# nsbuitrago/vfind

Measured on NVIDIA B200. Metric: reads/sec, higher is better.
Workload: dtype int32

## Files before the change

include/vfind_b200.h:

```cpp
#ifndef VFIND_B200_H
#define VFIND_B200_H

#include <stddef.h>
#include <stdint.h>

#ifdef __cplusplus
extern "C" {
#endif

#define VFB_ABI_VERSION 1

typedef enum vfb_status {
    VFB_OK = 0,
    VFB_ERR_VALUE = 1,
    VFB_ERR_IO = 2,
    VFB_ERR_FORMAT = 3,
    VFB_ERR_CUDA = 4,
    VFB_ERR_ARG = 5,
    VFB_ERR_NOMEM = 6
} vfb_status;

#define VFB_NONE 0xFFFFFFFFu

typedef struct vfb_params {
// ... 196 lines not shown
typedef struct vfb_dp_layout_info {
    int32_t packed;
    int32_t max_edits;
    int32_t accept_bound;
    uint32_t lcap;
    int32_t S0, LB, XB;
    int32_t c_eopen, c_eext, c_fopen, c_fext;
    int32_t hmask, lowmask, lenmask;
    int32_t neg_e, neg_f;
    int32_t w_match, w_mismatch, w_wild;
} vfb_dp_layout_info;

int vfb_debug_dp_layout(int32_t match_score, int32_t mismatch_score, int32_t gap_open_penalty, int32_t gap_extend_penalty,
                        uint32_t adapter_len, double accept_alignment, int32_t dp_mode, vfb_dp_layout_info *out);

int vfb_host_alloc(void **p, uint64_t bytes);
int vfb_host_free(void *p);

int vfb_pinned_pool_trim(void);
int vfb_device_pool_trim(void);

#ifdef __cplusplus
}
#endif
#endif
```

vfind_b200/csrc/api.cu:

```cuda
#include <cmath>
#include <cstdio>
#include <cstdlib>
#include <cstring>
#include <sched.h>
#include <string>
#include <thread>
#include <vector>

#include "hash.h"
#include "synth.h"
#include "ctx.cuh"

namespace vfb {

thread_local std::string g_error;
thread_local uint64_t g_launches = 0;

void set_error(const std::string &msg) { g_error = msg; }

int cuda_fail(cudaError_t e, const char *what, const char *file, int line)
{
    char buf[512];
    snprintf(buf, sizeof buf, "CUDA error %d (%s) at %s:%d: %s", (int)e, cudaGetErrorString(e), file, line, what);
    g_error = buf;
// ... 610 lines not shown
    if (c->st_parse) cudaStreamSynchronize(c->st_parse);
    for (auto &ln : c->lanes) { if (ln.st) cudaStreamSynchronize(ln.st); if (ln.st_dp) cudaStreamSynchronize(ln.st_dp); }
    for (auto &s : c->slots) {
        s.d_text.release(); s.d_spans.release(); s.h_text.release(); s.h_spans.release();
        if (s.copied) cudaEventDestroy(s.copied);
        for (auto &ev : s.computed) if (ev) cudaEventDestroy(ev);
    }
    for (auto &g : c->seg) {
        g.text.release(); g.z.release(); g.members.release(); g.spans.release();
        if (g.parsed) cudaEventDestroy(g.parsed);
        if (g.inflated) cudaEventDestroy(g.inflated);
        if (g.copied) cudaEventDestroy(g.copied);
        for (auto &ev : g.computed) if (ev) cudaEventDestroy(ev);
    }
    for (auto &ln : c->lanes) {
        DevBuf *lb[] = {&ln.d_start, &ln.d_end, &ln.d_list_a, &ln.d_list_b, &ln.d_fb_a, &ln.d_fb_b, &ln.d_c32, &ln.d_t64, &ln.d_keys,
                        &ln.d_koff, &ln.d_klen, &ln.d_khash, &ln.d_owner, &ln.d_wins, &ln.d_bestkey, &ln.d_cbval, &ln.d_fb2};
        for (auto *b : lb) b->release();
        if (ln.done) cudaEventDestroy(ln.done);
        if (ln.ev_scanned) cudaEventDestroy(ln.ev_scanned);
        if (ln.ev_aligned) cudaEventDestroy(ln.ev_aligned);
        if (ln.st) cudaStreamDestroy(ln.st);
        if (ln.st_dp) cudaStreamDestroy(ln.st_dp);
    }
    if (c->ev_fork) cudaEventDestroy(c->ev_fork);
    if (c->ev_k4) cudaEventDestroy(c->ev_k4);
    DevBuf *bufs[] = {&c->d_code_pre, &c->d_code_suf, &c->d_generic_scratch, &c->d_diag_exact_pre, &c->d_diag_exact_suf, &c->d_diag_score_pre,
                      &c->d_diag_len_pre, &c->d_diag_score_suf, &c->d_diag_len_suf, &c->t_slots,
                      &c->t_row_hash, &c->t_row_off, &c->t_row_len, &c->t_row_slot, &c->t_arena, &c->t_counters, &c->t_row_count,
                      &c->m_part_rows, &c->m_part_keys, &c->m_cursors, &c->m_chunk_off, &c->m_send, &c->m_recv,
                      &c->d_aligned_text, &c->d_span_sum,
                      &c->x_block_bytes, &c->x_block_rows, &c->x_offsets, &c->x_counts, &c->x_data,
// ... 144 lines not shown
    const uint64_t span_bytes_upper = span_len_ub;
    if (!text_bytes_hint) text_bytes_hint = span_bytes_upper;
    int rc;
    if (n == 0) return VFB_OK;
    const int li = c->n_lanes > 1 ? (int)(c->lane_seq++ & 1u) : 0;
    Lane &ln = c->lanes[li];
    cudaStream_t st = c->n_lanes > 1 ? ln.st : c->st_compute;
    if (lanes_used) *lanes_used |= 1u << li;
    const bool prof = c->profiling;
    if ((rc = ln.d_start.ensure((size_t)n * 4))) return rc;
    if ((rc = ln.d_end.ensure((size_t)n * 4))) return rc;
    if (c->align_pre) { if ((rc = ln.d_list_a.ensure((size_t)n * 4))) return rc; if ((rc = ln.d_fb_a.ensure((size_t)n * 4))) return rc; }
    if (c->align_suf) { if ((rc = ln.d_list_b.ensure((size_t)n * 4))) return rc; if ((rc = ln.d_fb_b.ensure((size_t)n * 4))) return rc; }
    const uint64_t key_bytes_ub = (c->prm.skip_translation ? span_bytes_upper : span_bytes_upper / 3) + 16ull * n;
    if ((rc = ln.d_keys.ensure(key_bytes_ub))) return rc;
    if ((rc = ln.d_koff.ensure((size_t)n * 8))) return rc;
    if ((rc = ln.d_klen.ensure((size_t)n * 4))) return rc;
    if ((rc = ln.d_khash.ensure((size_t)n * 8))) return rc;
    if ((rc = ln.d_owner.ensure((size_t)n * 4))) return rc;
    if (c->win_k_pre >= 0 || c->win_k_suf >= 0) {
        const uint32_t cap = n < 0x3FFFFFFFu ? n * 2u + 1024u : 0x7FFFFFFFu;
        if ((rc = ln.d_wins.ensure((size_t)cap * dpw_item_bytes()))) return rc;
        ln.win_cap = (uint32_t)(ln.d_wins.cap / dpw_item_bytes());
        if (c->prm.debug_win_cap > 0 && (uint32_t)c->prm.debug_win_cap < ln.win_cap) ln.win_cap = (uint32_t)c->prm.debug_win_cap;
        if ((rc = ln.d_bestkey.ensure((size_t)n * 8))) return rc;
        if ((rc = ln.d_cbval.ensure((size_t)n * 8))) return rc;
        if ((rc = ln.d_fb2.ensure((size_t)n * 4))) return rc;
    }
    const bool diag = c->prm.diagnostics != 0;
    if (diag) {
// ... 46 lines not shown
    ++g_launches;
    if (split) {
        VFB_CUDA(cudaEventRecord(ln.ev_aligned, sd));
        VFB_CUDA(cudaStreamWaitEvent(st, ln.ev_aligned, 0));
    }

    KeyJob kj;
    kj.text = d_text; kj.spans = d_spans;
    kj.start = ln.d_start.as<uint32_t>(); kj.end = ln.d_end.as<uint32_t>();
    kj.n_reads = n; kj.text_bytes = text_bytes_hint; kj.skip_translation = c->prm.skip_translation;
    kj.keys = ln.d_keys.as<uint8_t>(); kj.koff = ln.d_koff.as<uint64_t>();
    kj.key_cursor = ln.d_t64.as<unsigned long long>() + T_KEYBYTES;
    kj.klen = ln.d_klen.as<uint32_t>(); kj.khash = ln.d_khash.as<uint64_t>();
    kj.hash_bits = c->prm.debug_hash_bits;
    kj.flank_bytes = (uint32_t)(c->prefix.size() + c->suffix.size());
    bool k4_waited = false;
    InsertJob ij;
    ij.keys = kj.keys; ij.klen = kj.klen; ij.khash = kj.khash; ij.kcount = nullptr; ij.koff = kj.koff;
    ij.key_stride = 0; ij.n_keys = n; ij.owner_slot = ln.d_owner.as<uint32_t>();
    int frc = -1;
    if (c->fused_count && c->ub_rows > 0) {
        if (c->n_lanes > 1 && c->k4_pending) { VFB_CUDA(cudaStreamWaitEvent(st, c->ev_k4, 0)); k4_waited = true; }
        frc = launch_keys_count(kj, c->tab, ln.d_c32.as<uint32_t>() + C_NMISS, st);
        if (frc > 0) return frc;
        if (frc == VFB_OK) { ij.n_keys_dev = ln.d_c32.as<uint32_t>() + C_NMISS; ++c->stats.fused_batches; }
    }
    if (frc != VFB_OK && (rc = launch_keys(kj, st))) return rc;
    if (prof) VFB_CUDA(cudaEventRecord(pev[6], st));

    if (c->n_lanes > 1 && c->k4_pending && !k4_waited) VFB_CUDA(cudaStreamWaitEvent(st, c->ev_k4, 0));
    if ((rc = launch_insert(c->tab, ij, st))) return rc;
    if ((rc = snaps_push(c, n, key_bytes_ub, st))) return rc;
    if (c->n_lanes > 1) {
        VFB_CUDA(cudaEventRecord(c->ev_k4, st));
// ... 929 lines not shown
    DpLayout l;
    uint32_t lcap = 0;
    int K = -1;
    out->packed = plan_packed_dp(sc, adapter_len, out->accept_bound, dp_mode != 1, &l, &lcap, &K) ? 1 : 0;
    out->max_edits = out->packed ? K : -1;
    if (!out->packed) return VFB_OK;
    out->S0 = l.S0; out->LB = l.LB; out->XB = l.XB;
    out->c_eopen = l.c_eopen; out->c_eext = l.c_eext; out->c_fopen = l.c_fopen; out->c_fext = l.c_fext;
    out->hmask = l.hmask; out->lowmask = l.lowmask; out->lenmask = l.lenmask;
    out->neg_e = l.neg_e; out->neg_f = l.neg_f;
    out->w_match = l.w_match; out->w_mismatch = l.w_mismatch; out->w_wild = l.w_wild;
    out->lcap = lcap;
    return VFB_OK;
}

int vfb_host_alloc(void **p, uint64_t bytes)
{
    if (!p) { set_error("null argument"); return VFB_ERR_ARG; }
    VFB_CUDA(cudaMallocHost(p, bytes ? bytes : 1));
    return VFB_OK;
}

int vfb_host_free(void *p)
{
    if (p) VFB_CUDA(cudaFreeHost(p));
    return VFB_OK;
}

int vfb_pinned_pool_trim(void)
{
// ... 12 lines not shown
```

vfind_b200/csrc/ctx.cuh:

```cuda
#pragma once
#include <chrono>
#include <string>
#include <vector>

#include "vfb_internal.cuh"

namespace vfb {

void *device_acquire(int device, size_t want, size_t *cap_out);
void device_release(int device, void *p, size_t cap);
void device_pool_trim();

struct DevBuf {
    void *p = nullptr;
    size_t cap = 0;
    int dev = -1;
    int ensure(size_t bytes, bool keep = false, cudaStream_t st = 0)
    {
        if (bytes <= cap) return VFB_OK;
        if (dev < 0) VFB_CUDA(cudaGetDevice(&dev));
        const size_t want = bytes + bytes / 4 + 256;
        size_t ncap = 0;
        void *np = device_acquire(dev, want, &ncap);
        if (!np) {
// ... 37 lines not shown
    {
        pinned_release(p, cap);
        p = nullptr;
        cap = 0;
    }
};

#define VFB_LANES 2
struct Lane {
    cudaStream_t st = nullptr;
    cudaStream_t st_dp = nullptr;
    cudaEvent_t ev_scanned = nullptr, ev_aligned = nullptr;
    cudaEvent_t done = nullptr;
    bool pending = false;
    DevBuf d_start, d_end, d_list_a, d_list_b, d_fb_a, d_fb_b, d_c32, d_t64;
    DevBuf d_keys, d_koff, d_klen, d_khash, d_owner;
    DevBuf d_wins, d_bestkey, d_cbval, d_fb2;
    uint32_t win_cap = 0;
};

struct Slot {
    DevBuf d_text, d_spans;
    PinBuf h_text, h_spans;
    cudaEvent_t copied = nullptr, computed[VFB_LANES] = {nullptr, nullptr};
    unsigned busy = 0;
};

#define VFB_SEG_SLOTS 3
struct SegSlot {
    DevBuf text, z, members, spans;
    cudaEvent_t copied = nullptr, inflated = nullptr, parsed = nullptr;
    bool used = false;
    cudaEvent_t computed[VFB_LANES] = {nullptr, nullptr};
    unsigned busy = 0;
    uint64_t text_bytes = 0, z_bytes = 0;
    uint32_t n_members = 0;
};

enum { C_NPRE = 0, C_NSUF, C_FBPRE, C_FBSUF, C_FB2PRE, C_FB2SUF, C_NWINPRE, C_NWINSUF,
       C_WORKPRE = 32, C_WORKPRE2 = 64, C_WORKSUF = 96, C_WORKSUF2 = 128,
       C_NMISS = 160,
       C_COUNT32 = 192 };
enum { T_CELLS = 0, T_DPPRE, T_DPSUF, T_KEYBYTES, T_CELLSCOMP, T_WINDOWS, T_COUNT64 };

}

struct vfb_ctx {
    vfb_params prm;
    std::string prefix, suffix;
    vfb::AdapterBytes ad_pre, ad_suf;
    vfb::DpScoring sc;
    bool align_pre = false, align_suf = false;
    int min_accept_pre = 0, min_accept_suf = 0;
    bool packed_pre = false, packed_suf = false;
    vfb::DpLayout lay_pre, lay_suf;
    uint32_t lcap_pre = 0, lcap_suf = 0;
    vfb::DevBuf d_code_pre, d_code_suf;
// ... 74 lines not shown
```

vfind_b200/csrc/kernels_count.cu:

```cuda
#include "hash.h"
#include "translate_fast.h"
#include "vfb_internal.cuh"

namespace vfb {

__constant__ char c_aa[65] =
    "KNKN" "TTTT" "RSRS" "IIMI"
    "QHQH" "PPPP" "RRRR" "LLLL"
    "EDED" "AAAA" "GGGG" "VVVV"
    "*Y*Y" "SSSS" "*CWC" "LFLF";

__device__ __forceinline__ uint32_t tr_index(uint8_t b)
{
    switch (b) {
    case 'A': case 'a': return 0;
    case 'C': case 'c': return 1;
    case 'G': case 'g': return 2;
    case 'T': case 't': case 'U': case 'u': return 3;
    default: return 4;
    }
}

__device__ bool utf8_valid(const uint8_t *s, uint32_t n)
{
// ... 15 lines not shown
            if (i + 3 >= n) return false;
            const uint8_t b1 = s[i + 1], b2 = s[i + 2], b3 = s[i + 3];
            if ((b1 & 0xC0) != 0x80 || (b2 & 0xC0) != 0x80 || (b3 & 0xC0) != 0x80) return false;
            if (b == 0xF0 && b1 < 0x90) return false;
            if (b == 0xF4 && b1 > 0x8F) return false;
            i += 4;
        } else {
            return false;
        }
    }
    return true;
}

#define KEY_MULTS 128

#define K3T_WARPS_MAX 8
#define K3T_OUT_BYTES 4096
#define K3T_SLACK 16

struct Key3Tables {
    uint8_t lut25[256], lut5[256], lut1[256];
    uint8_t aa[128];
    uint64_t mult[KEY_MULTS];
};

__device__ __forceinline__ uint32_t k3_smem_u32(const void *p) { return (uint32_t)__cvta_generic_to_shared(p); }

template <bool SMEM>
__device__ __forceinline__ uint32_t k3_word(const uint32_t *w, uint32_t idx, const uint32_t *limit)
{
    if (SMEM) return w[idx];
    return (w + idx) < limit ? __ldg(w + idx) : 0u;
}

template <bool SMEM, bool TRANSLATE>
__device__ __forceinline__ uint64_t k3_lane(const Key3Tables &T, const uint32_t *w, const uint32_t *limit, uint32_t sh,
                                            uint32_t kl, uint32_t *out, uint32_t &high)
{
    const uint32_t nw = (kl + 3) >> 2, npad = ((kl + 15u) & ~15u) >> 2;
    uint64_t acc = 0;
    uint32_t t0 = k3_word<SMEM>(w, 0, limit), wp = 1;
// ... 15 lines not shown
            word = __funnelshift_r(t0, t1, sh);
            t0 = t1;
        }
        const uint32_t left = kl - 4 * wi;
        if (left < 4) word &= (1u << (8 * left)) - 1u;
        if (!TRANSLATE) high |= word & 0x80808080u;
        acc += (uint64_t)(word ^ VFB_HASH_K) * (wi < KEY_MULTS ? T.mult[wi] : vfb_hash_mult(wi));
        out[wi] = word;
    }
    for (uint32_t wi = nw; wi < npad; ++wi) out[wi] = 0u;
    return acc;
}

template <bool TRANSLATE>
__global__ void __launch_bounds__(K3T_WARPS_MAX * 32)
k3_keys_tile(const __grid_constant__ KeyJob job, const uint32_t tile_bytes)
{
    extern __shared__ __align__(128) uint8_t dyn[];
    __shared__ Key3Tables T;
    __shared__ unsigned long long bars[K3T_WARPS_MAX];
    for (int i = threadIdx.x; i < 256; i += blockDim.x) {
        const uint32_t c = i >= 128 ? 4u : tr_index((uint8_t)i);
        T.lut25[i] = (uint8_t)(25u * c); T.lut5[i] = (uint8_t)(5u * c); T.lut1[i] = (uint8_t)c;
    }
    for (int i = threadIdx.x; i < 128; i += blockDim.x) {
        const int c0 = i / 25, c1 = (i / 5) % 5, c2 = i % 5;
        T.aa[i] = (i >= 125 || c0 == 4 || c1 == 4 || c2 == 4) ? (uint8_t)'X' : (uint8_t)c_aa[c0 * 16 + c1 * 4 + c2];
    }
    for (int i = threadIdx.x; i < KEY_MULTS; i += blockDim.x) T.mult[i] = vfb_hash_mult((uint32_t)i);
    const int lane = threadIdx.x & 31, warp = threadIdx.x >> 5, n_warps = blockDim.x >> 5;
    if (lane == 0) {
        asm volatile("mbarrier.init.shared::cta.b64 [%0], 1;" ::"r"(k3_smem_u32(bars + warp)));
        asm volatile("fence.mbarrier_init.release.cluster;" ::: "memory");
    }
    __syncthreads();

    const size_t per_warp = (size_t)tile_bytes + K3T_SLACK + K3T_OUT_BYTES;
    uint8_t *tile = dyn + (size_t)warp * per_warp;
    const uint32_t *tile32 = reinterpret_cast<const uint32_t *>(tile);
    uint32_t *out32 = reinterpret_cast<uint32_t *>(tile + tile_bytes + K3T_SLACK);
    const uint32_t bar = k3_smem_u32(bars + warp), tile_s = k3_smem_u32(tile);
    uint32_t parity = 0;
    const uint32_t n_units = (job.n_reads + 31) / 32;
    for (uint32_t unit = blockIdx.x * n_warps + warp; unit < n_units; unit += gridDim.x * n_warps) {
        const uint32_t r = unit * 32 + lane;
        uint32_t klen = 0, V = 0, roff = 0;
        if (r < job.n_reads) {
            const uint32_t s = job.start[r], e = job.end[r];
            if (s != VFB_NONE && e != VFB_NONE && s < e) {
                const vfb_span sp = job.spans[r];
                if (e <= sp.len) {
                    V = e - s;
                    roff = sp.off + s;
                    if (!TRANSLATE) klen = V;
                    else if (V % 3 == 0) klen = V / 3;
                }
            }
        }
        const unsigned owners = __ballot_sync(0xffffffffu, klen != 0);
        if (owners == 0) {
            if (r < job.n_reads) job.klen[r] = 0;
            continue;
        }
        const uint32_t padded = (klen + 15u) & ~15u;
        uint32_t incl = padded;
#pragma unroll
        for (int o = 1; o < 32; o <<= 1) {
            const uint32_t t = __shfl_up_sync(0xffffffffu, incl, o);
            if (lane >= o) incl += t;
        }
        unsigned long long base = 0;
        const uint32_t total = __shfl_sync(0xffffffffu, incl, 31);
        if (lane == 31) base = atomicAdd(job.key_cursor, (unsigned long long)total);
        base = __shfl_sync(0xffffffffu, base, 31);
        const uint32_t local = incl - padded;
        const uint32_t lo = __reduce_min_sync(0xffffffffu, klen ? roff : 0xFFFFFFFFu);
        const uint32_t last = __reduce_max_sync(0xffffffffu, klen ? roff + (V - 1) : 0u);
        const uintptr_t g0 = reinterpret_cast<uintptr_t>(job.text + lo);
        const uint32_t lead_tile = (uint32_t)(g0 & 15u);
        const uint64_t n_bytes = ((uint64_t)(last - lo) + 1 + lead_tile + 15) & ~15ull;
        const bool staged = n_bytes <= tile_bytes;
        const bool out_staged = total <= K3T_OUT_BYTES;
        __syncwarp();
        if (staged) {
            if (lane == 0) {
                asm volatile("mbarrier.arrive.expect_tx.shared::cta.b64 _, [%0], %1;" ::"r"(bar), "r"((uint32_t)n_bytes) : "memory");
                asm volatile("cp.async.bulk.shared::cluster.global.mbarrier::complete_tx::bytes [%0], [%1], %2, [%3];"
                             ::"r"(tile_s), "l"(g0 & ~(uintptr_t)15), "r"((uint32_t)n_bytes), "r"(bar) : "memory");
            }
            uint32_t ok;
            do {
                asm volatile("{\n.reg .pred p;\nmbarrier.try_wait.parity.shared::cta.b64 p, [%1], %2;\nselp.u32 %0, 1, 0, p;\n}"
                             : "=r"(ok) : "r"(bar), "r"(parity) : "memory");
            } while (!ok);
            parity ^= 1u;
        }
        uint64_t acc = 0;
        uint32_t high = 0;
        if (klen) {
            uint32_t *out = out_staged ? out32 + (local >> 2) : reinterpret_cast<uint32_t *>(job.keys + base + local);
            if (staged) {
                const uint32_t toff = lead_tile + (roff - lo);
                acc = k3_lane<true, TRANSLATE>(T, tile32 + (toff >> 2), nullptr, (toff & 3u) * 8u, klen, out, high);
            } else {
                const uintptr_t va = reinterpret_cast<uintptr_t>(job.text + roff);
                const uint32_t *limit = reinterpret_cast<const uint32_t *>((va + V + 3) & ~(uintptr_t)3);
                acc = k3_lane<false, TRANSLATE>(T, reinterpret_cast<const uint32_t *>(va & ~(uintptr_t)3), limit,
                                                (uint32_t)(va & 3u) * 8u, klen, out, high);
            }
        }
        __syncwarp();
        if (out_staged) {
            const uint4 *src = reinterpret_cast<const uint4 *>(out32);
            uint4 *dst = reinterpret_cast<uint4 *>(job.keys + base);
            for (uint32_t c = lane; c < total / 16; c += 32) dst[c] = src[c];
        }
        if (klen) {
            job.koff[r] = base + local;
            uint64_t h = vfb_hash_finish(acc, klen);
            if (job.hash_bits > 0 && job.hash_bits < 64) h &= (1ull << job.hash_bits) - 1;
            job.khash[r] = h;
            if (!TRANSLATE && high && !utf8_valid(job.text + roff, V)) klen = 0;
        }
        if (r < job.n_reads) job.klen[r] = klen;
    }
}

static constexpr size_t keys_tile_block_smem(size_t tile, int w)
{
    return (size_t)w * (tile + K3T_SLACK + K3T_OUT_BYTES) + sizeof(Key3Tables) + 64 + 1024;
}
static_assert(keys_tile_block_smem(VFB_TILE_BYTES_MAX, 1) <= VFB_SMEM_BLOCK_MAX, "a block of one warp fits any tile");

template <bool TRANSLATE>
static int launch_keys_tile(const KeyJob &job, cudaStream_t st)
{
    const uint32_t tile = vfb_tile_bytes_for(job.text_bytes, job.n_reads);
    int best_w = 1, best_total = 0;
    for (int w = K3T_WARPS_MAX; w >= 1; w >>= 1) {
        int bps = (int)(VFB_SMEM_BLOCK_MAX / keys_tile_block_smem(tile, w));
        if (bps * w > 32) bps = 32 / w;
        if (bps * w > best_total) { best_total = bps * w; best_w = w; }
    }
    const size_t smem = (size_t)best_w * (tile + K3T_SLACK + K3T_OUT_BYTES);
    VFB_CUDA(cudaFuncSetAttribute(k3_keys_tile<TRANSLATE>, cudaFuncAttributeMaxDynamicSharedMemorySize, (int)smem));
    const uint32_t units = (job.n_reads + 31) / 32;
    uint32_t blocks = (units + best_w - 1) / best_w;
    const uint32_t cap = 148u * (uint32_t)(best_total / best_w);
    if (blocks > cap) blocks = cap;
    k3_keys_tile<TRANSLATE><<<blocks, best_w * 32, smem, st>>>(job, tile);
    return VFB_OK;
}

int launch_keys(const KeyJob &job, cudaStream_t st)
{
    if (job.n_reads == 0) return VFB_OK;
    const int rc = job.skip_translation ? launch_keys_tile<false>(job, st) : launch_keys_tile<true>(job, st);
    if (rc != VFB_OK) return rc;
    ++g_launches;
    VFB_CUDA(cudaGetLastError());
    return VFB_OK;
}

#define REF_BATCH 0x80000000u

// ... 210 lines not shown
            const uint4 *src = reinterpret_cast<const uint4 *>(key);
            uint4 *dst = reinterpret_cast<uint4 *>(job.keys + ko);
            for (uint32_t c = 0; c < padded / 16; ++c) dst[c] = src[c];
        }
        job.koff[m] = ko;
        job.klen[m] = klen;
        job.khash[m] = h;
    }
}

#define K34_WARPS_MAX 16

template <bool TRANSLATE>
__global__ void __maxnreg__(128)
k34_keys_count(const __grid_constant__ KeyJob job, const __grid_constant__ DevTable tab, uint32_t *n_miss,
               const uint32_t tile_bytes, const uint32_t out_bytes)
{
    extern __shared__ __align__(128) uint8_t dyn[];
    __shared__ Key34Tables T;
    __shared__ unsigned long long bars[K34_WARPS_MAX];
    for (int i = threadIdx.x; i < 256; i += blockDim.x) {
        const uint32_t c = i >= 128 ? 4u : tr_index((uint8_t)i);
        T.k3.lut25[i] = (uint8_t)(25u * c); T.k3.lut5[i] = (uint8_t)(5u * c); T.k3.lut1[i] = (uint8_t)c;
    }
    for (int i = threadIdx.x; i < 128; i += blockDim.x) {
        const int c0 = i / 25, c1 = (i / 5) % 5, c2 = i % 5;
        T.k3.aa[i] = (i >= 125 || c0 == 4 || c1 == 4 || c2 == 4) ? (uint8_t)'X' : (uint8_t)c_aa[c0 * 16 + c1 * 4 + c2];
    }
    for (int i = threadIdx.x; i < KEY_MULTS; i += blockDim.x) T.k3.mult[i] = vfb_hash_mult((uint32_t)i);
    for (int i = threadIdx.x; i < 4096; i += blockDim.x) T.codon[i] = tf_codon_entry((uint32_t)i, c_aa);
    for (int i = threadIdx.x; i < K34_AGG; i += blockDim.x) { T.agg_slot[i] = VFB_NONE; T.agg_cnt[i] = 0u; }
    const int lane = threadIdx.x & 31, warp = threadIdx.x >> 5, n_warps = blockDim.x >> 5;
    if (lane == 0) {
        asm volatile("mbarrier.init.shared::cta.b64 [%0], 1;" ::"r"(k3_smem_u32(bars + warp)));
        asm volatile("fence.mbarrier_init.release.cluster;" ::: "memory");
    }
    __syncthreads();

    const size_t per_warp = (size_t)tile_bytes + K3T_SLACK + 3 * (size_t)out_bytes + K34_STAGE_BYTES;
    uint8_t *tile = dyn + (size_t)warp * per_warp;
    const uint32_t *tile32 = reinterpret_cast<const uint32_t *>(tile);
    uint8_t *ring = tile + tile_bytes + K3T_SLACK;
    uint8_t *slot_land = ring + 3 * (size_t)out_bytes + (size_t)lane * 32;
    uint8_t *row_land = ring + 3 * (size_t)out_bytes + 32 * 32 + (size_t)lane * K34_ROW_BYTES;
    const uint32_t bar = k3_smem_u32(bars + warp), tile_s = k3_smem_u32(tile);
    const uint32_t slot_land_s = k3_smem_u32(slot_land), row_land_s = k3_smem_u32(row_land);
    const uint64_t mask = tab.capacity - 1;
    uint32_t parity = 0;
    uint32_t my_hits = 0;
    const uint32_t n_units = (job.n_reads + 31) / 32;
    const uint32_t stride = gridDim.x * n_warps;

    struct Plan {
        uint32_t klen, V, roff;
        uint32_t lo, n_bytes, lead;
        bool owners, staged;
    };
    auto make_plan = [&](bool in_range, uint32_t s, uint32_t e, vfb_span sp) {
        Plan p;
        p.klen = 0; p.V = 0; p.roff = 0;
        if (in_range && s != VFB_NONE && e != VFB_NONE && s < e && e <= sp.len) {
            p.V = e - s;
            p.roff = sp.off + s;
            if (!TRANSLATE) p.klen = p.V;
            else if (p.V % 3 == 0) p.klen = p.V / 3;
        }
        p.owners = __ballot_sync(0xffffffffu, p.klen != 0) != 0;
        p.lo = __reduce_min_sync(0xffffffffu, p.klen ? p.roff : 0xFFFFFFFFu);
        const uint32_t last = __reduce_max_sync(0xffffffffu, p.klen ? p.roff + (p.V - 1) : 0u);
        p.lead = (uint32_t)(reinterpret_cast<uintptr_t>(job.text + p.lo) & 15u);
        const uint64_t nb = ((uint64_t)(last - p.lo) + 1 + p.lead + 15) & ~15ull;
        p.staged = p.owners && nb <= tile_bytes;
        p.n_bytes = (uint32_t)nb;
        return p;
    };
    auto issue_tile = [&](const Plan &p) {
        if (p.staged && lane == 0) {
            const uintptr_t g0 = reinterpret_cast<uintptr_t>(job.text + p.lo);
            asm volatile("mbarrier.arrive.expect_tx.shared::cta.b64 _, [%0], %1;" ::"r"(bar), "r"(p.n_bytes) : "memory");
            asm volatile("cp.async.bulk.shared::cluster.global.mbarrier::complete_tx::bytes [%0], [%1], %2, [%3];"
                         ::"r"(tile_s), "l"(g0 & ~(uintptr_t)15), "r"(p.n_bytes), "r"(bar) : "memory");
        }
    };

    uint32_t unit = blockIdx.x * n_warps + warp;
    Plan cur;
    {
        const uint32_t r = unit * 32 + lane;
        const bool in = unit < n_units && r < job.n_reads;
        uint32_t s = VFB_NONE, e = VFB_NONE;
        vfb_span sp; sp.off = 0; sp.len = 0;
        if (in) { s = job.start[r]; e = job.end[r]; sp = job.spans[r]; }
        cur = make_plan(in, s, e, sp);
        issue_tile(cur);
    }
    uint64_t h1 = 0, h2 = 0;
    uint32_t klen1 = 0, klen2 = 0, kpos1 = 0, kpos2 = 0;
    uint32_t st1 = 0, st2 = 0;
    uint32_t slot2 = 0;
    unsigned rsv_mask = 0;
    uint32_t rsv_m0 = 0, rsv_rank = 0, rsv_off = 0;
    unsigned long long rsv_base = 0;
    bool any1 = false, any2 = false;
    uint32_t bi = 0;

    for (;; unit += stride) {
        const bool live = unit < n_units;
        if (!live && !any1 && !any2) break;
        __syncwarp();
        uint32_t ns = VFB_NONE, ne = VFB_NONE;
        vfb_span nsp; nsp.off = 0; nsp.len = 0;
        const uint32_t nr = (unit + stride) * 32 + lane;
        const bool n_in = live && unit + stride < n_units && nr < job.n_reads;
        if (n_in) { ns = job.start[nr]; ne = job.end[nr]; nsp = job.spans[nr]; }

        uint32_t klen = live ? cur.klen : 0u;
        const bool owners = live && cur.owners;
        uint64_t h = 0;
        uint32_t padded = 0, local = 0;
        bool out_staged = true;
        unsigned long long base = 0;
        uint32_t *out = nullptr;
        if (owners) {
            padded = (klen + 15u) & ~15u;
            uint32_t incl = padded;
#pragma unroll
            for (int o = 1; o < 32; o <<= 1) {
                const uint32_t t = __shfl_up_sync(0xffffffffu, incl, o);
                if (lane >= o) incl += t;
            }
            const uint32_t total = __shfl_sync(0xffffffffu, incl, 31);
            local = incl - padded;
            out_staged = total <= out_bytes;
            if (!out_staged) {
                if (lane == 31) base = atomicAdd(job.key_cursor, (unsigned long long)total);
                base = __shfl_sync(0xffffffffu, base, 31);
            }
            uint32_t *blk = reinterpret_cast<uint32_t *>(ring + (size_t)bi * out_bytes);
            out = out_staged ? blk + (local >> 2) : reinterpret_cast<uint32_t *>(job.keys + base + local);
            if (cur.staged) {
                uint32_t ok;
                do {
                    asm volatile("{\n.reg .pred p;\nmbarrier.try_wait.parity.shared::cta.b64 p, [%1], %2;\nselp.u32 %0, 1, 0, p;\n}"
                                 : "=r"(ok) : "r"(bar), "r"(parity) : "memory");
                } while (!ok);
                parity ^= 1u;
            }
            if (klen) {
                uint64_t acc;
                uint32_t high = 0;
                if (cur.staged) {
                    const uint32_t toff = cur.lead + (cur.roff - cur.lo);
                    if (TRANSLATE && out_staged && klen <= 128u)
                        acc = k34_lane_hot(T, tile32 + (toff >> 2), (toff & 3u) * 8u, klen, blk + (local >> 2));
                    else if (TRANSLATE) acc = k34_lane_translate<true>(T, tile32 + (toff >> 2), nullptr, (toff & 3u) * 8u, klen, out);
                    else acc = k3_lane<true, false>(T.k3, tile32 + (toff >> 2), nullptr, (toff & 3u) * 8u, klen, out, high);
                } else {
                    const uintptr_t va = reinterpret_cast<uintptr_t>(job.text + cur.roff);
                    const uint32_t *limit = reinterpret_cast<const uint32_t *>((va + cur.V + 3) & ~(uintptr_t)3);
                    const uint32_t *w = reinterpret_cast<const uint32_t *>(va & ~(uintptr_t)3);
                    if (TRANSLATE) acc = k34_lane_translate<false>(T, w, limit, (uint32_t)(va & 3u) * 8u, klen, out);
                    else acc = k3_lane<false, false>(T.k3, w, limit, (uint32_t)(va & 3u) * 8u, klen, out, high);
                }
                h = vfb_hash_finish(acc, klen);
                if (job.hash_bits > 0 && job.hash_bits < 64) h &= (1ull << job.hash_bits) - 1;
                if (!TRANSLATE && high && !utf8_valid(job.text + cur.roff, cur.V)) klen = 0;
            }
        }
        __syncwarp();
        const Plan nxt = make_plan(n_in, ns, ne, nsp);
        issue_tile(nxt);

        asm volatile("cp.async.wait_all;" ::: "memory");
        if (any2) {
            const uint32_t *key2 = reinterpret_cast<const uint32_t *>(ring + kpos2);
            bool late = false;
            if (st2 == 2u) {
                const uint4 *row = reinterpret_cast<const uint4 *>(row_land);
                const uint4 *key = reinterpret_cast<const uint4 *>(key2);
                const uint32_t n16 = (klen2 + 15u) >> 4;
                uint32_t diff = 0;
#pragma unroll
                for (uint32_t c = 0; c < K34_ROW_BYTES / 16; ++c)
                    if (c < n16) {
                        const uint4 u = row[c], v = key[c];
                        diff |= (u.x ^ v.x) | (u.y ^ v.y) | (u.z ^ v.z) | (u.w ^ v.w);
// ... 87 lines not shown
        for (int o = 16; o > 0; o >>= 1) hits += __shfl_xor_sync(0xffffffffu, hits, o);
        if (lane == 0 && hits) {
            atomicAdd(&tab.counters[2], (unsigned long long)hits);
            atomicAdd(&tab.counters[3], (unsigned long long)hits);
        }
    }
    __syncthreads();
    for (int e = threadIdx.x; e < K34_AGG; e += blockDim.x)
        if (T.agg_slot[e] != VFB_NONE && T.agg_cnt[e])
            atomicAdd(&tab.slots[(uint64_t)T.agg_slot[e] * VFB_SLOT_WORDS + 1], (unsigned long long)T.agg_cnt[e]);
}

template <bool TRANSLATE>
static int launch_keys_count_t(const KeyJob &job, const DevTable &tab, uint32_t *n_miss, cudaStream_t st)
{
    const uint32_t tile = vfb_tile_bytes_for(job.text_bytes, job.n_reads);
    const uint64_t stride = job.n_reads ? job.text_bytes / job.n_reads : 0;
    const uint64_t region_ub = stride > job.flank_bytes ? stride - job.flank_bytes : 0;
    const uint64_t key_ub = TRANSLATE ? region_ub / 3 : region_ub;
    uint32_t out_bytes = (uint32_t)(32 * ((key_ub + 15) & ~15ull));
    if (out_bytes < 1024) out_bytes = 1024;
    if (out_bytes > 4096u) out_bytes = 4096u;
    const size_t per_warp = (size_t)tile + K3T_SLACK + 3 * (size_t)out_bytes + K34_STAGE_BYTES;
    int best_w = 0, best_total = 0;
    for (int w = K34_WARPS_MAX; w >= 1; --w) {
        const size_t per_block = (size_t)w * per_warp + sizeof(Key34Tables) + 8 * K34_WARPS_MAX + 1024;
        int bps = (int)(VFB_SMEM_BLOCK_MAX / per_block);
        if (bps * w > 16) bps = 16 / w;
        if (bps * w > best_total) { best_total = bps * w; best_w = w; }
    }
    if (best_total == 0) return -1;
    const size_t smem = (size_t)best_w * per_warp;
    VFB_CUDA(cudaFuncSetAttribute(k34_keys_count<TRANSLATE>, cudaFuncAttributeMaxDynamicSharedMemorySize, (int)smem));
    const uint32_t units = (job.n_reads + 31) / 32;
    uint32_t blocks = (units + best_w - 1) / best_w;
    const uint32_t cap = 148u * (uint32_t)(best_total / best_w);
    if (blocks > cap) blocks = cap;
    k34_keys_count<TRANSLATE><<<blocks, best_w * 32, smem, st>>>(job, tab, n_miss, tile, out_bytes);
    return VFB_OK;
}

int launch_keys_count(const KeyJob &job, const DevTable &tab, uint32_t *n_miss, cudaStream_t st)
{
    if (job.n_reads == 0 || job.text_bytes == 0) return -1;
    const int rc = job.skip_translation ? launch_keys_count_t<false>(job, tab, n_miss, st)
                                        : launch_keys_count_t<true>(job, tab, n_miss, st);
    if (rc != VFB_OK) return rc;
    ++g_launches;
    VFB_CUDA(cudaGetLastError());
    return VFB_OK;
}

#define INS_THREADS 256
// ... 515 lines not shown
```

vfind_b200/csrc/vfb_internal.cuh:

```cuda
#pragma once
#include <cuda_runtime.h>
#include <stdint.h>

#include <string>

#include "../../include/vfind_b200.h"

#define VFB_MAX_PACKED_ADAPTER 64
#define VFB_MAX_ADAPTER 1024
#define VFB_MAX_SCAN_ADAPTER 256

namespace vfb {

void set_error(const std::string &msg);
bool trace_on();
void trace(const char *fmt, ...);
int cuda_fail(cudaError_t e, const char *what, const char *file, int line);
void *pinned_acquire(size_t want, size_t *cap_out);
void pinned_release(void *p, size_t cap);
void pinned_pool_trim();

#define VFB_CUDA(call)                                                         \
    do {                                                                       \
        cudaError_t e__ = (call);                                              \
// ... 86 lines not shown
    int force_general;
};
#define VFB_TILE_BYTES_MAX (96u * 1024u)
#define VFB_SMEM_BLOCK_MAX (227u * 1024u)
uint32_t vfb_tile_bytes_for(uint64_t text_bytes, uint32_t n_reads);
int launch_scan(const ScanJob &job, const AdapterBytes &prefix, const AdapterBytes &suffix,
                int sm_count, cudaStream_t st);

struct KeyJob {
    const uint8_t *text;
    const vfb_span *spans;
    const uint32_t *start, *end;
    uint32_t n_reads;
    uint64_t text_bytes;
    int skip_translation;
    uint8_t *keys;
    uint64_t *koff;
    unsigned long long *key_cursor;
    uint32_t *klen;
    uint64_t *khash;
    int hash_bits;
    uint32_t flank_bytes;
};
int launch_keys(const KeyJob &job, cudaStream_t st);
struct DevTable;
int launch_keys_count(const KeyJob &job, const DevTable &tab, uint32_t *n_miss, cudaStream_t st);

#define VFB_SLOT_WORDS 4
struct DevTable {
    unsigned long long *slots;
    uint64_t capacity;
    uint64_t *row_hash;
    uint64_t *row_off;
    uint32_t *row_len;
    uint32_t *row_slot;
    uint64_t row_capacity;
    uint8_t *arena;
    uint64_t arena_capacity;
// ... 101 lines not shown
```

Baseline: 2.181 billion.

## Compact keyed reads into a list and stage per-lane text slots via bulk copies

Adds a stream-compaction kernel that writes the indices of reads with a valid variable region into a dense list, so the key and fused key-count kernels only walk keyed reads instead of every read. The per-warp contiguous TMA tile covering the whole span of 32 reads is replaced by per-lane fixed-size slots, each filled with its own bulk copy of just that read's region, sized from the average read stride. This is meant to cut wasted staging bytes and idle lanes on unkeyed reads. In exchange it adds an extra kernel launch, a device-side list count read by each kernel, and outputs indexed by list position rather than read index, which downstream insert code must handle through n_keys_dev.

```diff
diff --git a/include/vfind_b200.h b/include/vfind_b200.h
--- a/include/vfind_b200.h
+++ b/include/vfind_b200.h
@@ -234,6 +234,8 @@
 int vfb_debug_dp_layout(int32_t match_score, int32_t mismatch_score, int32_t gap_open_penalty, int32_t gap_extend_penalty,
                         uint32_t adapter_len, double accept_alignment, int32_t dp_mode, vfb_dp_layout_info *out);
 
+uint32_t vfb_debug_key_slot_bytes(uint64_t text_bytes, uint32_t n_reads, uint32_t flank_bytes);
+
 int vfb_host_alloc(void **p, uint64_t bytes);
 int vfb_host_free(void *p);
 
diff --git a/vfind_b200/csrc/api.cu b/vfind_b200/csrc/api.cu
--- a/vfind_b200/csrc/api.cu
+++ b/vfind_b200/csrc/api.cu
@@ -648,8 +648,8 @@
         for (auto &ev : g.computed) if (ev) cudaEventDestroy(ev);
     }
     for (auto &ln : c->lanes) {
-        DevBuf *lb[] = {&ln.d_start, &ln.d_end, &ln.d_list_a, &ln.d_list_b, &ln.d_fb_a, &ln.d_fb_b, &ln.d_c32, &ln.d_t64, &ln.d_keys,
-                        &ln.d_koff, &ln.d_klen, &ln.d_khash, &ln.d_owner, &ln.d_wins, &ln.d_bestkey, &ln.d_cbval, &ln.d_fb2};
+        DevBuf *lb[] = {&ln.d_start, &ln.d_end, &ln.d_list_a, &ln.d_list_b, &ln.d_fb_a, &ln.d_fb_b, &ln.d_c32, &ln.d_t64, &ln.d_klist,
+                        &ln.d_keys, &ln.d_koff, &ln.d_klen, &ln.d_khash, &ln.d_owner, &ln.d_wins, &ln.d_bestkey, &ln.d_cbval, &ln.d_fb2};
         for (auto *b : lb) b->release();
         if (ln.done) cudaEventDestroy(ln.done);
         if (ln.ev_scanned) cudaEventDestroy(ln.ev_scanned);
@@ -824,6 +824,7 @@
     if (c->align_suf) { if ((rc = ln.d_list_b.ensure((size_t)n * 4))) return rc; if ((rc = ln.d_fb_b.ensure((size_t)n * 4))) return rc; }
     const uint64_t key_bytes_ub = (c->prm.skip_translation ? span_bytes_upper : span_bytes_upper / 3) + 16ull * n;
     if ((rc = ln.d_keys.ensure(key_bytes_ub))) return rc;
+    if ((rc = ln.d_klist.ensure((size_t)n * 4))) return rc;
     if ((rc = ln.d_koff.ensure((size_t)n * 8))) return rc;
     if ((rc = ln.d_klen.ensure((size_t)n * 4))) return rc;
     if ((rc = ln.d_khash.ensure((size_t)n * 8))) return rc;
@@ -900,10 +901,12 @@
     kj.klen = ln.d_klen.as<uint32_t>(); kj.khash = ln.d_khash.as<uint64_t>();
     kj.hash_bits = c->prm.debug_hash_bits;
     kj.flank_bytes = (uint32_t)(c->prefix.size() + c->suffix.size());
+    kj.list = ln.d_klist.as<uint32_t>(); kj.n_list = ln.d_c32.as<uint32_t>() + C_NKEYED;
+    if ((rc = launch_key_list(kj, st))) return rc;
     bool k4_waited = false;
     InsertJob ij;
     ij.keys = kj.keys; ij.klen = kj.klen; ij.khash = kj.khash; ij.kcount = nullptr; ij.koff = kj.koff;
-    ij.key_stride = 0; ij.n_keys = n; ij.owner_slot = ln.d_owner.as<uint32_t>();
+    ij.key_stride = 0; ij.n_keys = n; ij.n_keys_dev = kj.n_list; ij.owner_slot = ln.d_owner.as<uint32_t>();
     int frc = -1;
     if (c->fused_count && c->ub_rows > 0) {
         if (c->n_lanes > 1 && c->k4_pending) { VFB_CUDA(cudaStreamWaitEvent(st, c->ev_k4, 0)); k4_waited = true; }
@@ -1863,6 +1866,11 @@
     return VFB_OK;
 }
 
+uint32_t vfb_debug_key_slot_bytes(uint64_t text_bytes, uint32_t n_reads, uint32_t flank_bytes)
+{
+    return key_slot_bytes_for(text_bytes, n_reads, flank_bytes);
+}
+
 int vfb_host_alloc(void **p, uint64_t bytes)
 {
     if (!p) { set_error("null argument"); return VFB_ERR_ARG; }
diff --git a/vfind_b200/csrc/ctx.cuh b/vfind_b200/csrc/ctx.cuh
--- a/vfind_b200/csrc/ctx.cuh
+++ b/vfind_b200/csrc/ctx.cuh
@@ -75,7 +75,7 @@
     cudaEvent_t done = nullptr;
     bool pending = false;
     DevBuf d_start, d_end, d_list_a, d_list_b, d_fb_a, d_fb_b, d_c32, d_t64;
-    DevBuf d_keys, d_koff, d_klen, d_khash, d_owner;
+    DevBuf d_klist, d_keys, d_koff, d_klen, d_khash, d_owner;
     DevBuf d_wins, d_bestkey, d_cbval, d_fb2;
     uint32_t win_cap = 0;
 };
@@ -101,7 +101,8 @@
 enum { C_NPRE = 0, C_NSUF, C_FBPRE, C_FBSUF, C_FB2PRE, C_FB2SUF, C_NWINPRE, C_NWINSUF,
        C_WORKPRE = 32, C_WORKPRE2 = 64, C_WORKSUF = 96, C_WORKSUF2 = 128,
        C_NMISS = 160,
-       C_COUNT32 = 192 };
+       C_NKEYED = 192,
+       C_COUNT32 = 224 };
 enum { T_CELLS = 0, T_DPPRE, T_DPSUF, T_KEYBYTES, T_CELLSCOMP, T_WINDOWS, T_COUNT64 };
 
 }
diff --git a/vfind_b200/csrc/kernels_count.cu b/vfind_b200/csrc/kernels_count.cu
--- a/vfind_b200/csrc/kernels_count.cu
+++ b/vfind_b200/csrc/kernels_count.cu
@@ -53,9 +53,72 @@
 
 #define KEY_MULTS 128
 
+#define KL_THREADS 256
+#define KL_ITEMS 8
+
+__global__ void __launch_bounds__(KL_THREADS)
+k3_key_list(const uint32_t *start, const uint32_t *end, const vfb_span *spans, uint32_t n_reads, int translate,
+            uint32_t *list, uint32_t *n_list)
+{
+    constexpr int W = KL_THREADS / 32;
+    __shared__ uint32_t s_pos[KL_ITEMS * W];
+    const int lane = threadIdx.x & 31, warp = threadIdx.x >> 5;
+    const uint32_t base = blockIdx.x * (KL_THREADS * KL_ITEMS);
+    unsigned ball[KL_ITEMS];
+    uint32_t s[KL_ITEMS], e[KL_ITEMS], len[KL_ITEMS];
+#pragma unroll
+    for (int k = 0; k < KL_ITEMS; ++k) {
+        const uint32_t r = base + k * KL_THREADS + threadIdx.x;
+        s[k] = VFB_NONE; e[k] = VFB_NONE; len[k] = 0;
+        if (r < n_reads) { s[k] = start[r]; e[k] = end[r]; len[k] = spans[r].len; }
+    }
+#pragma unroll
+    for (int k = 0; k < KL_ITEMS; ++k) {
+        const bool keyed = s[k] != VFB_NONE && e[k] != VFB_NONE && s[k] < e[k] && e[k] <= len[k] &&
+                           (!translate || (e[k] - s[k]) % 3 == 0);
+        ball[k] = __ballot_sync(0xffffffffu, keyed);
+        if (lane == 0) s_pos[k * W + warp] = (uint32_t)__popc(ball[k]);
+    }
+    __syncthreads();
+    if (warp == 0) {
+        static_assert(KL_ITEMS * W == 64, "warp 0 scans two counts per lane");
+        const uint32_t c0 = s_pos[2 * lane], c1 = s_pos[2 * lane + 1];
+        uint32_t incl = c0 + c1;
+#pragma unroll
+        for (int o = 1; o < 32; o <<= 1) {
+            const uint32_t t = __shfl_up_sync(0xffffffffu, incl, o);
+            if (lane >= o) incl += t;
+        }
+        uint32_t first = 0;
+        if (lane == 31 && incl) first = atomicAdd(n_list, incl);
+        first = __shfl_sync(0xffffffffu, first, 31);
+        const uint32_t excl = first + incl - (c0 + c1);
+        s_pos[2 * lane] = excl;
+        s_pos[2 * lane + 1] = excl + c0;
+    }
+    __syncthreads();
+#pragma unroll
+    for (int k = 0; k < KL_ITEMS; ++k)
+        if ((ball[k] >> lane) & 1u)
+            list[s_pos[k * W + warp] + __popc(ball[k] & ((1u << lane) - 1u))] = base + k * KL_THREADS + threadIdx.x;
+}
+
+int launch_key_list(const KeyJob &job, cudaStream_t st)
+{
+    if (job.n_reads == 0) return VFB_OK;
+    const uint32_t per_block = KL_THREADS * KL_ITEMS;
+    const uint32_t blocks = (uint32_t)(((uint64_t)job.n_reads + per_block - 1) / per_block);
+    k3_key_list<<<blocks, KL_THREADS, 0, st>>>(job.start, job.end, job.spans, job.n_reads, job.skip_translation ? 0 : 1,
+                                               job.list, job.n_list);
+    ++g_launches;
+    VFB_CUDA(cudaGetLastError());
+    return VFB_OK;
+}
+
 #define K3T_WARPS_MAX 8
 #define K3T_OUT_BYTES 4096
 #define K3T_SLACK 16
+#define K3_SLOT_MIN 64
 
 struct Key3Tables {
     uint8_t lut25[256], lut5[256], lut1[256];
@@ -64,6 +127,34 @@
 };
 
 __device__ __forceinline__ uint32_t k3_smem_u32(const void *p) { return (uint32_t)__cvta_generic_to_shared(p); }
+
+__device__ __forceinline__ uint32_t k3_cover(const uint8_t *g, uint32_t V, uint32_t slot_bytes)
+{
+    const uint64_t nb = ((uint64_t)(reinterpret_cast<uintptr_t>(g) & 15u) + V + 15) & ~15ull;
+    return nb <= slot_bytes ? (uint32_t)nb : 0u;
+}
+
+__device__ __forceinline__ bool k3_stage(uint32_t bar, uint32_t slot_s, const uint8_t *g, uint32_t n_bytes)
+{
+    const uint32_t total = __reduce_add_sync(0xffffffffu, n_bytes);
+    if (total == 0) return false;
+    if ((threadIdx.x & 31) == 0)
+        asm volatile("mbarrier.arrive.expect_tx.shared::cta.b64 _, [%0], %1;" ::"r"(bar), "r"(total) : "memory");
+    if (n_bytes)
+        asm volatile("cp.async.bulk.shared::cluster.global.mbarrier::complete_tx::bytes [%0], [%1], %2, [%3];"
+                     ::"r"(slot_s), "l"(reinterpret_cast<uintptr_t>(g) & ~(uintptr_t)15), "r"(n_bytes), "r"(bar) : "memory");
+    return true;
+}
+
+__device__ __forceinline__ void k3_wait(uint32_t bar, uint32_t &parity)
+{
+    uint32_t ok;
+    do {
+        asm volatile("{\n.reg .pred p;\nmbarrier.try_wait.parity.shared::cta.b64 p, [%1], %2;\nselp.u32 %0, 1, 0, p;\n}"
+                     : "=r"(ok) : "r"(bar), "r"(parity) : "memory");
+    } while (!ok);
+    parity ^= 1u;
+}
 
 template <bool SMEM>
 __device__ __forceinline__ uint32_t k3_word(const uint32_t *w, uint32_t idx, const uint32_t *limit)
@@ -109,7 +200,7 @@
 
 template <bool TRANSLATE>
 __global__ void __launch_bounds__(K3T_WARPS_MAX * 32)
-k3_keys_tile(const __grid_constant__ KeyJob job, const uint32_t tile_bytes)
+k3_keys_tile(const __grid_constant__ KeyJob job, const uint32_t slot_bytes)
 {
     extern __shared__ __align__(128) uint8_t dyn[];
     __shared__ Key3Tables T;
@@ -130,32 +221,24 @@
     }
     __syncthreads();
 
+    const uint32_t tile_bytes = 32 * slot_bytes;
     const size_t per_warp = (size_t)tile_bytes + K3T_SLACK + K3T_OUT_BYTES;
     uint8_t *tile = dyn + (size_t)warp * per_warp;
     const uint32_t *tile32 = reinterpret_cast<const uint32_t *>(tile);
     uint32_t *out32 = reinterpret_cast<uint32_t *>(tile + tile_bytes + K3T_SLACK);
-    const uint32_t bar = k3_smem_u32(bars + warp), tile_s = k3_smem_u32(tile);
+    const uint32_t bar = k3_smem_u32(bars + warp), slot_s = k3_smem_u32(tile + (size_t)lane * slot_bytes);
     uint32_t parity = 0;
-    const uint32_t n_units = (job.n_reads + 31) / 32;
+    const uint32_t n_list = *job.n_list;
+    const uint32_t n_units = (n_list + 31) / 32;
     for (uint32_t unit = blockIdx.x * n_warps + warp; unit < n_units; unit += gridDim.x * n_warps) {
-        const uint32_t r = unit * 32 + lane;
-        uint32_t klen = 0, V = 0, roff = 0;
-        if (r < job.n_reads) {
-            const uint32_t s = job.start[r], e = job.end[r];
-            if (s != VFB_NONE && e != VFB_NONE && s < e) {
-                const vfb_span sp = job.spans[r];
-                if (e <= sp.len) {
-                    V = e - s;
-                    roff = sp.off + s;
-                    if (!TRANSLATE) klen = V;
-                    else if (V % 3 == 0) klen = V / 3;
-                }
-            }
-        }
-        const unsigned owners = __ballot_sync(0xffffffffu, klen != 0);
-        if (owners == 0) {
-            if (r < job.n_reads) job.klen[r] = 0;
-            continue;
+        const uint32_t p = unit * 32 + lane;
+        uint32_t klen = 0, V = 0, roff = 0, n_bytes = 0;
+        if (p < n_list) {
+            const uint32_t r = job.list[p], s = job.start[r];
+            V = job.end[r] - s;
+            roff = job.spans[r].off + s;
+            klen = TRANSLATE ? V / 3 : V;
+            n_bytes = k3_cover(job.text + roff, V, slot_bytes);
         }
         const uint32_t padded = (klen + 15u) & ~15u;
         uint32_t incl = padded;
@@ -169,36 +252,18 @@
         if (lane == 31) base = atomicAdd(job.key_cursor, (unsigned long long)total);
         base = __shfl_sync(0xffffffffu, base, 31);
         const uint32_t local = incl - padded;
-        const uint32_t lo = __reduce_min_sync(0xffffffffu, klen ? roff : 0xFFFFFFFFu);
-        const uint32_t last = __reduce_max_sync(0xffffffffu, klen ? roff + (V - 1) : 0u);
-        const uintptr_t g0 = reinterpret_cast<uintptr_t>(job.text + lo);
-        const uint32_t lead_tile = (uint32_t)(g0 & 15u);
-        const uint64_t n_bytes = ((uint64_t)(last - lo) + 1 + lead_tile + 15) & ~15ull;
-        const bool staged = n_bytes <= tile_bytes;
         const bool out_staged = total <= K3T_OUT_BYTES;
         __syncwarp();
-        if (staged) {
-            if (lane == 0) {
-                asm volatile("mbarrier.arrive.expect_tx.shared::cta.b64 _, [%0], %1;" ::"r"(bar), "r"((uint32_t)n_bytes) : "memory");
-                asm volatile("cp.async.bulk.shared::cluster.global.mbarrier::complete_tx::bytes [%0], [%1], %2, [%3];"
-                             ::"r"(tile_s), "l"(g0 & ~(uintptr_t)15), "r"((uint32_t)n_bytes), "r"(bar) : "memory");
-            }
-            uint32_t ok;
-            do {
-                asm volatile("{\n.reg .pred p;\nmbarrier.try_wait.parity.shared::cta.b64 p, [%1], %2;\nselp.u32 %0, 1, 0, p;\n}"
-                             : "=r"(ok) : "r"(bar), "r"(parity) : "memory");
-            } while (!ok);
-            parity ^= 1u;
-        }
+        if (k3_stage(bar, slot_s, job.text + roff, n_bytes)) k3_wait(bar, parity);
         uint64_t acc = 0;
         uint32_t high = 0;
         if (klen) {
             uint32_t *out = out_staged ? out32 + (local >> 2) : reinterpret_cast<uint32_t *>(job.keys + base + local);
-            if (staged) {
-                const uint32_t toff = lead_tile + (roff - lo);
+            const uintptr_t va = reinterpret_cast<uintptr_t>(job.text + roff);
+            if (n_bytes) {
+                const uint32_t toff = lane * slot_bytes + (uint32_t)(va & 15u);
                 acc = k3_lane<true, TRANSLATE>(T, tile32 + (toff >> 2), nullptr, (toff & 3u) * 8u, klen, out, high);
             } else {
-                const uintptr_t va = reinterpret_cast<uintptr_t>(job.text + roff);
                 const uint32_t *limit = reinterpret_cast<const uint32_t *>((va + V + 3) & ~(uintptr_t)3);
                 acc = k3_lane<false, TRANSLATE>(T, reinterpret_cast<const uint32_t *>(va & ~(uintptr_t)3), limit,
                                                 (uint32_t)(va & 3u) * 8u, klen, out, high);
@@ -211,13 +276,13 @@
             for (uint32_t c = lane; c < total / 16; c += 32) dst[c] = src[c];
         }
         if (klen) {
-            job.koff[r] = base + local;
+            job.koff[p] = base + local;
             uint64_t h = vfb_hash_finish(acc, klen);
             if (job.hash_bits > 0 && job.hash_bits < 64) h &= (1ull << job.hash_bits) - 1;
-            job.khash[r] = h;
+            job.khash[p] = h;
             if (!TRANSLATE && high && !utf8_valid(job.text + roff, V)) klen = 0;
-        }
-        if (r < job.n_reads) job.klen[r] = klen;
+            job.klen[p] = klen;
+        }
     }
 }
 
@@ -226,11 +291,28 @@
     return (size_t)w * (tile + K3T_SLACK + K3T_OUT_BYTES) + sizeof(Key3Tables) + 64 + 1024;
 }
 static_assert(keys_tile_block_smem(VFB_TILE_BYTES_MAX, 1) <= VFB_SMEM_BLOCK_MAX, "a block of one warp fits any tile");
+
+static uint64_t region_bytes_expected(uint64_t text_bytes, uint32_t n_reads, uint32_t flank_bytes)
+{
+    const uint64_t stride = n_reads ? text_bytes / n_reads : 0;
+    return stride > flank_bytes ? stride - flank_bytes : 0;
+}
+
+uint32_t key_slot_bytes_for(uint64_t text_bytes, uint32_t n_reads, uint32_t flank_bytes)
+{
+    const uint64_t stride = n_reads ? text_bytes / n_reads : 0;
+    uint64_t s = (stride + 15 + 15) & ~15ull;
+    if (s < K3_SLOT_MIN) s = K3_SLOT_MIN;
+    if (s > VFB_TILE_BYTES_MAX / 32) s = VFB_TILE_BYTES_MAX / 32;
+    return (uint32_t)s;
+}
+
+static uint32_t key_slot_bytes(const KeyJob &job) { return key_slot_bytes_for(job.text_bytes, job.n_reads, job.flank_bytes); }
 
 template <bool TRANSLATE>
 static int launch_keys_tile(const KeyJob &job, cudaStream_t st)
 {
-    const uint32_t tile = vfb_tile_bytes_for(job.text_bytes, job.n_reads);
+    const uint32_t slot = key_slot_bytes(job), tile = 32 * slot;
     int best_w = 1, best_total = 0;
     for (int w = K3T_WARPS_MAX; w >= 1; w >>= 1) {
         int bps = (int)(VFB_SMEM_BLOCK_MAX / keys_tile_block_smem(tile, w));
@@ -243,7 +325,7 @@
     uint32_t blocks = (units + best_w - 1) / best_w;
     const uint32_t cap = 148u * (uint32_t)(best_total / best_w);
     if (blocks > cap) blocks = cap;
-    k3_keys_tile<TRANSLATE><<<blocks, best_w * 32, smem, st>>>(job, tile);
+    k3_keys_tile<TRANSLATE><<<blocks, best_w * 32, smem, st>>>(job, slot);
     return VFB_OK;
 }
 
@@ -484,7 +566,7 @@
 template <bool TRANSLATE>
 __global__ void __maxnreg__(128)
 k34_keys_count(const __grid_constant__ KeyJob job, const __grid_constant__ DevTable tab, uint32_t *n_miss,
-               const uint32_t tile_bytes, const uint32_t out_bytes)
+               const uint32_t slot_bytes, const uint32_t out_bytes)
 {
     extern __shared__ __align__(128) uint8_t dyn[];
     __shared__ Key34Tables T;
@@ -507,63 +589,51 @@
     }
     __syncthreads();
 
+    const uint32_t tile_bytes = 32 * slot_bytes;
     const size_t per_warp = (size_t)tile_bytes + K3T_SLACK + 3 * (size_t)out_bytes + K34_STAGE_BYTES;
     uint8_t *tile = dyn + (size_t)warp * per_warp;
     const uint32_t *tile32 = reinterpret_cast<const uint32_t *>(tile);
     uint8_t *ring = tile + tile_bytes + K3T_SLACK;
     uint8_t *slot_land = ring + 3 * (size_t)out_bytes + (size_t)lane * 32;
     uint8_t *row_land = ring + 3 * (size_t)out_bytes + 32 * 32 + (size_t)lane * K34_ROW_BYTES;
-    const uint32_t bar = k3_smem_u32(bars + warp), tile_s = k3_smem_u32(tile);
+    const uint32_t bar = k3_smem_u32(bars + warp), text_slot_s = k3_smem_u32(tile + (size_t)lane * slot_bytes);
     const uint32_t slot_land_s = k3_smem_u32(slot_land), row_land_s = k3_smem_u32(row_land);
     const uint64_t mask = tab.capacity - 1;
     uint32_t parity = 0;
     uint32_t my_hits = 0;
-    const uint32_t n_units = (job.n_reads + 31) / 32;
+    const uint32_t n_list = *job.n_list;
+    const uint32_t n_units = (n_list + 31) / 32;
     const uint32_t stride = gridDim.x * n_warps;
 
     struct Plan {
         uint32_t klen, V, roff;
-        uint32_t lo, n_bytes, lead;
+        uint32_t n_bytes;
         bool owners, staged;
     };
-    auto make_plan = [&](bool in_range, uint32_t s, uint32_t e, vfb_span sp) {
+    auto make_plan = [&](bool in, uint32_t s, uint32_t e, uint32_t off) {
         Plan p;
-        p.klen = 0; p.V = 0; p.roff = 0;
-        if (in_range && s != VFB_NONE && e != VFB_NONE && s < e && e <= sp.len) {
+        p.klen = 0; p.V = 0; p.roff = 0; p.n_bytes = 0;
+        if (in) {
             p.V = e - s;
-            p.roff = sp.off + s;
-            if (!TRANSLATE) p.klen = p.V;
-            else if (p.V % 3 == 0) p.klen = p.V / 3;
+            p.roff = off + s;
+            p.klen = TRANSLATE ? p.V / 3 : p.V;
+            p.n_bytes = k3_cover(job.text + p.roff, p.V, slot_bytes);
         }
         p.owners = __ballot_sync(0xffffffffu, p.klen != 0) != 0;
-        p.lo = __reduce_min_sync(0xffffffffu, p.klen ? p.roff : 0xFFFFFFFFu);
-        const uint32_t last = __reduce_max_sync(0xffffffffu, p.klen ? p.roff + (p.V - 1) : 0u);
-        p.lead = (uint32_t)(reinterpret_cast<uintptr_t>(job.text + p.lo) & 15u);
-        const uint64_t nb = ((uint64_t)(last - p.lo) + 1 + p.lead + 15) & ~15ull;
-        p.staged = p.owners && nb <= tile_bytes;
-        p.n_bytes = (uint32_t)nb;
+        p.staged = k3_stage(bar, text_slot_s, job.text + p.roff, p.n_bytes);
         return p;
     };
-    auto issue_tile = [&](const Plan &p) {
-        if (p.staged && lane == 0) {
-            const uintptr_t g0 = reinterpret_cast<uintptr_t>(job.text + p.lo);
-            asm volatile("mbarrier.arrive.expect_tx.shared::cta.b64 _, [%0], %1;" ::"r"(bar), "r"(p.n_bytes) : "memory");
-            asm volatile("cp.async.bulk.shared::cluster.global.mbarrier::complete_tx::bytes [%0], [%1], %2, [%3];"
-                         ::"r"(tile_s), "l"(g0 & ~(uintptr_t)15), "r"(p.n_bytes), "r"(bar) : "memory");
-        }
-    };
+    auto listed = [&](uint32_t u) { return u < n_units && u * 32 + lane < n_list ? job.list[u * 32 + lane] : VFB_NONE; };
 
     uint32_t unit = blockIdx.x * n_warps + warp;
     Plan cur;
     {
-        const uint32_t r = unit * 32 + lane;
-        const bool in = unit < n_units && r < job.n_reads;
-        uint32_t s = VFB_NONE, e = VFB_NONE;
-        vfb_span sp; sp.off = 0; sp.len = 0;
-        if (in) { s = job.start[r]; e = job.end[r]; sp = job.spans[r]; }
-        cur = make_plan(in, s, e, sp);
-        issue_tile(cur);
-    }
+        const uint32_t r = listed(unit);
+        uint32_t s = 0, e = 0, off = 0;
+        if (r != VFB_NONE) { s = job.start[r]; e = job.end[r]; off = job.spans[r].off; }
+        cur = make_plan(r != VFB_NONE, s, e, off);
+    }
+    uint32_t r_next = listed(unit + stride);
     uint64_t h1 = 0, h2 = 0;
     uint32_t klen1 = 0, klen2 = 0, kpos1 = 0, kpos2 = 0;
     uint32_t st1 = 0, st2 = 0;
@@ -578,11 +648,10 @@
         const bool live = unit < n_units;
         if (!live && !any1 && !any2) break;
         __syncwarp();
-        uint32_t ns = VFB_NONE, ne = VFB_NONE;
-        vfb_span nsp; nsp.off = 0; nsp.len = 0;
-        const uint32_t nr = (unit + stride) * 32 + lane;
-        const bool n_in = live && unit + stride < n_units && nr < job.n_reads;
-        if (n_in) { ns = job.start[nr]; ne = job.end[nr]; nsp = job.spans[nr]; }
+        uint32_t ns = 0, ne = 0, noff = 0;
+        const bool n_in = r_next != VFB_NONE;
+        if (n_in) { ns = job.start[r_next]; ne = job.end[r_next]; noff = job.spans[r_next].off; }
+        r_next = listed(unit + 2 * stride);
 
         uint32_t klen = live ? cur.klen : 0u;
         const bool owners = live && cur.owners;
@@ -608,19 +677,12 @@
             }
             uint32_t *blk = reinterpret_cast<uint32_t *>(ring + (size_t)bi * out_bytes);
             out = out_staged ? blk + (local >> 2) : reinterpret_cast<uint32_t *>(job.keys + base + local);
-            if (cur.staged) {
-                uint32_t ok;
-                do {
-                    asm volatile("{\n.reg .pred p;\nmbarrier.try_wait.parity.shared::cta.b64 p, [%1], %2;\nselp.u32 %0, 1, 0, p;\n}"
-                                 : "=r"(ok) : "r"(bar), "r"(parity) : "memory");
-                } while (!ok);
-                parity ^= 1u;
-            }
+            if (cur.staged) k3_wait(bar, parity);
             if (klen) {
                 uint64_t acc;
                 uint32_t high = 0;
-                if (cur.staged) {
-                    const uint32_t toff = cur.lead + (cur.roff - cur.lo);
+                if (cur.n_bytes) {
+                    const uint32_t toff = lane * slot_bytes + (uint32_t)(reinterpret_cast<uintptr_t>(job.text + cur.roff) & 15u);
                     if (TRANSLATE && out_staged && klen <= 128u)
                         acc = k34_lane_hot(T, tile32 + (toff >> 2), (toff & 3u) * 8u, klen, blk + (local >> 2));
                     else if (TRANSLATE) acc = k34_lane_translate<true>(T, tile32 + (toff >> 2), nullptr, (toff & 3u) * 8u, klen, out);
@@ -638,8 +700,7 @@
             }
         }
         __syncwarp();
-        const Plan nxt = make_plan(n_in, ns, ne, nsp);
-        issue_tile(nxt);
+        const Plan nxt = make_plan(n_in, ns, ne, noff);
 
         asm volatile("cp.async.wait_all;" ::: "memory");
         if (any2) {
@@ -757,14 +818,13 @@
 template <bool TRANSLATE>
 static int launch_keys_count_t(const KeyJob &job, const DevTable &tab, uint32_t *n_miss, cudaStream_t st)
 {
-    const uint32_t tile = vfb_tile_bytes_for(job.text_bytes, job.n_reads);
-    const uint64_t stride = job.n_reads ? job.text_bytes / job.n_reads : 0;
-    const uint64_t region_ub = stride > job.flank_bytes ? stride - job.flank_bytes : 0;
-    const uint64_t key_ub = TRANSLATE ? region_ub / 3 : region_ub;
+    const uint32_t slot = key_slot_bytes(job);
+    const uint64_t region = region_bytes_expected(job.text_bytes, job.n_reads, job.flank_bytes);
+    const uint64_t key_ub = TRANSLATE ? region / 3 : region;
     uint32_t out_bytes = (uint32_t)(32 * ((key_ub + 15) & ~15ull));
     if (out_bytes < 1024) out_bytes = 1024;
     if (out_bytes > 4096u) out_bytes = 4096u;
-    const size_t per_warp = (size_t)tile + K3T_SLACK + 3 * (size_t)out_bytes + K34_STAGE_BYTES;
+    const size_t per_warp = (size_t)32 * slot + K3T_SLACK + 3 * (size_t)out_bytes + K34_STAGE_BYTES;
     int best_w = 0, best_total = 0;
     for (int w = K34_WARPS_MAX; w >= 1; --w) {
         const size_t per_block = (size_t)w * per_warp + sizeof(Key34Tables) + 8 * K34_WARPS_MAX + 1024;
@@ -779,7 +839,7 @@
     uint32_t blocks = (units + best_w - 1) / best_w;
     const uint32_t cap = 148u * (uint32_t)(best_total / best_w);
     if (blocks > cap) blocks = cap;
-    k34_keys_count<TRANSLATE><<<blocks, best_w * 32, smem, st>>>(job, tab, n_miss, tile, out_bytes);
+    k34_keys_count<TRANSLATE><<<blocks, best_w * 32, smem, st>>>(job, tab, n_miss, slot, out_bytes);
     return VFB_OK;
 }
 
diff --git a/vfind_b200/csrc/vfb_internal.cuh b/vfind_b200/csrc/vfb_internal.cuh
--- a/vfind_b200/csrc/vfb_internal.cuh
+++ b/vfind_b200/csrc/vfb_internal.cuh
@@ -124,6 +124,8 @@
     uint32_t n_reads;
     uint64_t text_bytes;
     int skip_translation;
+    uint32_t *list;
+    uint32_t *n_list;
     uint8_t *keys;
     uint64_t *koff;
     unsigned long long *key_cursor;
@@ -132,6 +134,8 @@
     int hash_bits;
     uint32_t flank_bytes;
 };
+int launch_key_list(const KeyJob &job, cudaStream_t st);
+uint32_t key_slot_bytes_for(uint64_t text_bytes, uint32_t n_reads, uint32_t flank_bytes);
 int launch_keys(const KeyJob &job, cudaStream_t st);
 struct DevTable;
 int launch_keys_count(const KeyJob &job, const DevTable &tab, uint32_t *n_miss, cudaStream_t st);
```

After: 2.263 billion (median of 6 runs). +3.8%, better.
